# dordanino12/unet-convlstm

Hardware: AMD Instinct MI355X
Metric: training frames/sec, Moving-MNIST 64x64 seq-20 (higher is better)
Workload: dtype bf16; 1 GPU; TemporalUNetDualView(base_ch=64, use_skip_lstm=True) train step, 64x64 seq-20, per-GPU batch 32, AdamW+clip; global_batch=32, seq_len=20, parallelism=dp1

## Files before the change

### include/uclstm.h

```cpp
#ifndef UCLSTM_H
#define UCLSTM_H

#include <stdint.h>

#ifdef __cplusplus
extern "C" {
#endif

#define UCLSTM_ABI_VERSION 16

#define UCLSTM_OK            0
#define UCLSTM_E_BADARG     -1
#define UCLSTM_E_LAUNCH     -2
#define UCLSTM_E_NODEVICE   -3

#define UCLSTM_ACT_TYPE_BF16 0
#define UCLSTM_ACT_TYPE_F16  1


typedef struct {
    const void* ptr;
    int32_t C;
    int32_t Hs, Ws;
    int32_t offY, offX;
// ... 213 lines not shown
                             const int32_t* argmax, void* dx, float* dw, int32_t dw_accumulate, float* scratch, int32_t n_img,
                             int32_t H, int32_t W, int32_t Cp, int32_t C, int32_t k, void* stream);

int32_t uclstm_colsum(const void* a, float* out, int64_t pixels, int32_t Cp, void* stream);
int64_t uclstm_colsum_ordered_rows(int64_t pixels, int32_t Cp);
int32_t uclstm_colsum_ordered(const void* a, float* partials, float* out, int64_t pixels, int32_t Cp, int32_t accumulate,
                              int32_t act_type, void* stream);
int32_t uclstm_ordered_sum_f32(const float* partials, int32_t rows, int32_t cols, float* out, int32_t accumulate, void* stream);
int32_t uclstm_ordered_sum_f64(const double* partials, int32_t rows, int32_t cols, double* out, int32_t accumulate, void* stream);

int32_t uclstm_loss_fwd(const float* y_pred, const float* y, const float* mask, double* sums,
                        int64_t planes, int32_t H, int32_t W, void* stream);
int64_t uclstm_loss_fwd_ordered_rows(int64_t planes, int32_t H, int32_t W);
int32_t uclstm_loss_fwd_ordered(const float* y_pred, const float* y, const float* mask, double* partials, double* sums,
                                int32_t accumulate, int64_t planes, int32_t H, int32_t W, void* stream);
int32_t uclstm_loss_bwd(const float* y_pred, const float* y, const float* mask, const float* coefs,
                        float* grad, int64_t planes, int32_t H, int32_t W, void* stream);

int32_t uclstm_sumsq(const float* g, int64_t n, double* out , void* stream);
int64_t uclstm_sumsq_ordered_rows(int64_t n);
int32_t uclstm_sumsq_ordered(const float* g, int64_t n, double* partials, double* out, int32_t accumulate, void* stream);
int32_t uclstm_adamw_step(float* p, float* m, float* v, const float* g, int64_t n, const double* sumsq, float max_norm,
                          float lr, float beta1, float beta2, float eps, float weight_decay, int32_t step, void* stream);

int32_t uclstm_adamw_step_dev(float* p, float* m, float* v, const float* g, int64_t n, const double* sumsq, float* hyper, void* stream);

int32_t uclstm_adamw_step_groups(float* p, float* m, float* v, const float* g, int64_t n, const double* sumsq,
                                 const int64_t* runs, int32_t n_runs, float* hyper, int32_t n_groups,
                                 const float* scale_state, void* stream);

int32_t uclstm_adamw_step_scaled(float* p, float* m, float* v, const float* g, int64_t n, const double* sumsq, float max_norm,
                                 float lr, float beta1, float beta2, float eps, float weight_decay, const float* scale_state,
                                 void* stream);
int32_t uclstm_loss_scale_update(float* scale_state, const double* sumsq, float growth, float backoff, int32_t interval,
                                 void* stream);

int32_t uclstm_dataset_transform(const float* x_raw, const float* y_raw, float* x, float* y, float* mask, int64_t n_frames,
                                 int32_t C, int32_t HW, float norm_const, float min_vel, float max_vel, int32_t clip,
                                 float y_scale, float trans_min, float trans_max, void* stream);
int32_t uclstm_dataset_gather_transform(const float* x_all, const float* y_all, const int64_t* idx, int64_t n_seq, int64_t n_out,
                                        int32_t T, int32_t C, int32_t HW, float* x, float* y, float* mask, int32_t transform,
                                        float norm_const, float min_vel, float max_vel, int32_t clip, float y_scale,
                                        float trans_min, float trans_max, void* stream);
int32_t uclstm_dataset_gather_augment(const float* x_all, const float* y_all, const int64_t* idx, const int32_t* aug,
        int64_t n_seq, int64_t n_out, int32_t T_src, int32_t T_out, int32_t C, int32_t Hs, int32_t Ws, int32_t Ho, int32_t Wo,
        int32_t flags, float* x, float* y, float* mask, int32_t transform, float norm_const, float min_vel, float max_vel, int32_t clip,
// ... 81 lines not shown
```

### unet-convlstm_amd/_lib.py

```python
from __future__ import annotations

import ctypes as C
import os
import re

import torch

HERE = os.path.dirname(os.path.abspath(__file__))
LIB_PATH = os.environ.get("UCLSTM_LIB") or os.path.join(HERE, "libuclstm.so")
HEADER_PATH = os.path.join(HERE, "..", "include", "uclstm.h")

ABI_VERSION = 16
EPI_STORE, EPI_LSTM, EPI_ATOMIC = 0, 1, 2
NMODE_IDENTITY, NMODE_LSTM, NMODE_TAPMAJOR = 0, 1, 2
KMODE_IDENTITY, KMODE_GATES, KMODE_IM2COL = 0, 1, 2
ACT_TYPE_BF16, ACT_TYPE_F16 = 0, 1

_ERRORS = {-1: "bad argument (shape/alignment/null contract)", -2: "kernel launch failed", -3: "no gfx950 device"}


class UclstmError(RuntimeError):
    pass


# ... 120 lines not shown
    "uclstm_nchw_grad_to_nhwc": [_P, _P, _I, _I, _I, _I, _I, _P],
    "uclstm_im2col3x3_first": [_P, _P, _I, _I, _I, _I, _I, _I, _L, _L, _P],
    "uclstm_nchw_to_nhwc_f32": [_P, _P, _I, _I, _I, _I, _I, _P],
    "uclstm_nhwc_to_nchw_f32": [_P, _P, _I, _I, _I, _I, _I, _P],
    "uclstm_outconv_fwd": [_P, _P, _P, _P, _L, _I, _I, _I, _I, _P],
    "uclstm_outconv_bwd": [_P, _P, _P, _P, _P, _P, _L, _I, _I, _I, _I, _P],
    "uclstm_outconv_bwd_ordered_rows": [_L, _I],
    "uclstm_outconv_bwd_ordered": [_P, _P, _P, _P, _P, _P, _P, _I, _L, _I, _I, _I, _I, _I, _P],
    "uclstm_colsum": [_P, _P, _L, _I, _P],
    "uclstm_colsum_ordered_rows": [_L, _I],
    "uclstm_colsum_ordered": [_P, _P, _P, _L, _I, _I, _I, _P],
    "uclstm_ordered_sum_f32": [_P, _I, _I, _P, _I, _P],
    "uclstm_ordered_sum_f64": [_P, _I, _I, _P, _I, _P],
    "uclstm_attention_fwd": [_P, _P, _P, _P, _P, _P, _I, _I, _I, _I, _I, _I, _P],
    "uclstm_attention_bwd": [_P, _P, _P, _P, _P, _P, _P, _P, _I, _P, _I, _I, _I, _I, _I, _I, _P],
    "uclstm_loss_fwd": [_P, _P, _P, _P, _L, _I, _I, _P],
    "uclstm_loss_fwd_ordered_rows": [_L, _I, _I],
    "uclstm_loss_fwd_ordered": [_P, _P, _P, _P, _P, _I, _L, _I, _I, _P],
    "uclstm_loss_bwd": [_P, _P, _P, _P, _P, _L, _I, _I, _P],
    "uclstm_sumsq": [_P, _L, _P, _P],
    "uclstm_sumsq_ordered_rows": [_L],
    "uclstm_sumsq_ordered": [_P, _L, _P, _P, _I, _P],
    "uclstm_adamw_step": [_P, _P, _P, _P, _L, _P, _F, _F, _F, _F, _F, _F, _I, _P],
    "uclstm_adamw_step_dev": [_P, _P, _P, _P, _L, _P, _P, _P],
    "uclstm_adamw_step_groups": [_P, _P, _P, _P, _L, _P, _P, _I, _P, _I, _P, _P],
    "uclstm_adamw_step_scaled": [_P, _P, _P, _P, _L, _P, _F, _F, _F, _F, _F, _F, _P, _P],
    "uclstm_loss_scale_update": [_P, _P, _F, _F, _I, _P],
    "uclstm_dataset_transform": [_P, _P, _P, _P, _P, _L, _I, _I, _F, _F, _F, _I, _F, _F, _F, _P],
    "uclstm_dataset_gather_transform": [_P, _P, _P, _L, _L, _I, _I, _I, _P, _P, _P, _I, _F, _F, _F, _I, _F, _F, _F, _P],
    "uclstm_dataset_gather_augment": [_P, _P, _P, _P, _L, _L, _I, _I, _I, _I, _I, _I, _I, _I, _P, _P, _P, _I, _F, _F, _F, _I, _F, _F, _F, _P],
    "uclstm_plane_d4": [_P, _P, _L, _I, _I, _I, _I, _F, _P],
    "uclstm_sprites_render": [_P, _I, _I, _I, _P, _L, _I, _I, _I, _I, _I, _F, _P, _P, _P, _P, _P],
    "uclstm_metric_sums": [_P, _P, _P, _P, _L, _F, _F, _F, _P],
    "uclstm_metric_sums_ordered_rows": [_L],
    "uclstm_metric_sums_ordered": [_P, _P, _P, _P, _P, _I, _L, _F, _F, _F, _P],
    "uclstm_eval_stats": [C.POINTER(EvalDesc), _P],
    "uclstm_eval_stats_rows": [_L, _L],
    "uclstm_stream_spin": [_I, _P],
    "uclstm_abi_version": [],
    "uclstm_build_arch": [],
    "uclstm_source_hash": [],
    "uclstm_last_error_string": [],
}
_RESTYPES = {"uclstm_build_arch": C.c_char_p, "uclstm_source_hash": C.c_char_p, "uclstm_last_error_string": C.c_char_p, "uclstm_bn_bwd_reduce_rows": C.c_int64, "uclstm_bn_pool_bwd_rows": C.c_int64,
             "uclstm_eval_stats_rows": C.c_int64, "uclstm_colsum_ordered_rows": C.c_int64, "uclstm_outconv_bwd_ordered_rows": C.c_int64,
             "uclstm_loss_fwd_ordered_rows": C.c_int64, "uclstm_sumsq_ordered_rows": C.c_int64, "uclstm_metric_sums_ordered_rows": C.c_int64}
# ... 73 lines not shown
```

### unet-convlstm_amd/csrc/common.h

```cpp
#pragma once
#include <hip/hip_runtime.h>
#include <stdint.h>

#if defined(UCLSTM_ACT_F16)
#define uclstm_igemm_fwd uclstm_igemm_fwd_f16
#define uclstm_igemm_fwd_group uclstm_igemm_fwd_group_f16
#define uclstm_igemm_wgrad uclstm_igemm_wgrad_f16
#define uclstm_pack_weights uclstm_pack_weights_f16
#define uclstm_pack_weights_batched uclstm_pack_weights_batched_f16
#define uclstm_splitk_finish uclstm_splitk_finish_f16
#define uclstm_bn_apply_relu uclstm_bn_apply_relu_f16
#define uclstm_bn_bwd_reduce uclstm_bn_bwd_reduce_f16
#define uclstm_bn_bwd_apply uclstm_bn_bwd_apply_f16
#define uclstm_bn_head_fwd uclstm_bn_head_fwd_f16
#define uclstm_bn_apply_relu_pool uclstm_bn_apply_relu_pool_f16
#define uclstm_bn_pool_bwd_reduce uclstm_bn_pool_bwd_reduce_f16
#define uclstm_bn_pool_bwd_apply uclstm_bn_pool_bwd_apply_f16
#define uclstm_bn_head_bwd_reduce uclstm_bn_head_bwd_reduce_f16
#define uclstm_bn_head_bwd_apply uclstm_bn_head_bwd_apply_f16
#define uclstm_maxpool2_fwd uclstm_maxpool2_fwd_f16
#define uclstm_maxpool2_bwd uclstm_maxpool2_bwd_f16
#define uclstm_lstm_bwd_pointwise uclstm_lstm_bwd_pointwise_f16
#define uclstm_lstm_fwd_pointwise uclstm_lstm_fwd_pointwise_f16
#define uclstm_lstm_fwd_pointwise_group uclstm_lstm_fwd_pointwise_group_f16
#define uclstm_nchw_to_nhwc uclstm_nchw_to_nhwc_f16
#define uclstm_nhwc_to_nchw uclstm_nhwc_to_nchw_f16
#define uclstm_nchw_grad_to_nhwc uclstm_nchw_grad_to_nhwc_f16
#define uclstm_im2col3x3_first uclstm_im2col3x3_first_f16
#define uclstm_outconv_fwd uclstm_outconv_fwd_f16
#define uclstm_outconv_bwd uclstm_outconv_bwd_f16
#define uclstm_colsum uclstm_colsum_f16
#define uclstm_attention_fwd uclstm_attention_fwd_f16
// ... 101 lines not shown
```

### unet-convlstm_amd/csrc/loss_optim.hip

```cpp
#include "common.h"

namespace {

constexpr int NT = 256;

__device__ __forceinline__ double wave_sum(double v) {
#pragma unroll
    for (int o = 32; o > 0; o >>= 1) v += __shfl_xor(v, o, 64);
    return v;
}

template <int K>
__device__ __forceinline__ void block_sum(double (&v)[K], double* red ) {
#pragma unroll
    for (int k = 0; k < K; ++k) v[k] = wave_sum(v[k]);
    const int lane = threadIdx.x & 63, wave = threadIdx.x >> 6;
    if (lane == 0)
#pragma unroll
        for (int k = 0; k < K; ++k) red[wave * K + k] = v[k];
    __syncthreads();
    if (threadIdx.x == 0)
#pragma unroll
        for (int k = 0; k < K; ++k) v[k] = red[k] + red[K + k] + red[2 * K + k] + red[3 * K + k];
}
// ... 86 lines not shown
    const int64_t n4 = n >> 2;
    const float4* g4 = (const float4*)g;
    for (int64_t i = (int64_t)blockIdx.x * NT + threadIdx.x; i < n4; i += (int64_t)gridDim.x * NT) {
        const float4 v = g4[i];
        acc[0] += (double)(v.x * v.x + v.y * v.y) + (double)(v.z * v.z + v.w * v.w);
    }
    if (blockIdx.x == 0 && threadIdx.x < (n & 3)) {
        const float v = g[(n4 << 2) + threadIdx.x];
        acc[0] += (double)(v * v);
    }
    if constexpr (ORDERED) {
        block_sum_store<1>(acc, red, out + blockIdx.x);
    } else {
        block_sum<1>(acc, red);
        if (threadIdx.x == 0) atomicAdd(out, acc[0]);
    }
}

__device__ __forceinline__ bool step_overflowed(double ss) { return !(fabs(ss) <= 1.7976931348623157e308); }

__global__ void adamw_kernel(float* __restrict__ p, float* __restrict__ m, float* __restrict__ v, const float* __restrict__ g,
                             int64_t n, const double* __restrict__ sumsq, float max_norm, float lr, float b1, float b2, float eps,
                             float wd, float inv_bc1, float inv_sqrt_bc2) {
    float coef = 1.f;
    if (sumsq && max_norm > 0.f) {
        const float total = (float)sqrt(*sumsq);
        coef = fminf(max_norm / (total + 1e-6f), 1.f);
    }
    for (int64_t i = (int64_t)blockIdx.x * NT + threadIdx.x; i < n; i += (int64_t)gridDim.x * NT) {
        const float gi = g[i] * coef;
        float w = p[i] * (1.f - lr * wd);
        const float mi = b1 * m[i] + (1.f - b1) * gi;
        const float vi = b2 * v[i] + (1.f - b2) * gi * gi;
        const float denom = sqrtf(vi) * inv_sqrt_bc2 + eps;
        w -= lr * inv_bc1 * mi / denom;
        p[i] = w;
        m[i] = mi;
        v[i] = vi;
    }
}

__global__ void adamw_dev_kernel(float* __restrict__ p, float* __restrict__ m, float* __restrict__ v, const float* __restrict__ g,
                                 int64_t n, const double* __restrict__ sumsq, const float* __restrict__ hyper) {
    const float lr = hyper[0], b1 = hyper[1], b2 = hyper[2], eps = hyper[3], wd = hyper[4], max_norm = hyper[5];
    const double step = (double)hyper[6] + 1.0;
    const float inv_bc1 = (float)(1.0 / (1.0 - pow((double)b1, step)));
    const float inv_sqrt_bc2 = (float)(1.0 / sqrt(1.0 - pow((double)b2, step)));
    float coef = 1.f;
    if (sumsq && max_norm > 0.f) {
        const float total = (float)sqrt(*sumsq);
        coef = fminf(max_norm / (total + 1e-6f), 1.f);
    }
    for (int64_t i = (int64_t)blockIdx.x * NT + threadIdx.x; i < n; i += (int64_t)gridDim.x * NT) {
        const float gi = g[i] * coef;
        float w = p[i] * (1.f - lr * wd);
        const float mi = b1 * m[i] + (1.f - b1) * gi;
        const float vi = b2 * v[i] + (1.f - b2) * gi * gi;
        const float denom = sqrtf(vi) * inv_sqrt_bc2 + eps;
// ... 321 lines not shown
    const int64_t total = planes * H * W;
    if (total >= ((int64_t)1 << 31)) return UCLSTM_E_BADARG;
    UCLSTM_LAUNCH(loss_bwd_kernel, dim3(grid_for(total, 2048)), dim3(NT), 0, (hipStream_t)stream, y_pred, y, mask, coefs, grad,
                       total, make_fastdiv(H * W), make_fastdiv(W), H, W);
    return UCLSTM_OK;
}

extern "C" int32_t uclstm_sumsq(const float* g, int64_t n, double* out, void* stream) {
    if (!g || !out || n <= 0 || ((uintptr_t)g % 16)) return UCLSTM_E_BADARG;
    UCLSTM_LAUNCH(sumsq_kernel<false>, dim3(grid_for((n + 3) / 4, 1024)), dim3(NT), 0, (hipStream_t)stream, g, n, out);
    return UCLSTM_OK;
}

extern "C" int32_t uclstm_adamw_step(float* p, float* m, float* v, const float* g, int64_t n, const double* sumsq, float max_norm,
                                     float lr, float beta1, float beta2, float eps, float weight_decay, int32_t step, void* stream) {
    if (!p || !m || !v || !g || n <= 0 || step < 1) return UCLSTM_E_BADARG;
    const double bc1 = 1.0 - pow((double)beta1, (double)step);
    const double bc2 = 1.0 - pow((double)beta2, (double)step);
    UCLSTM_LAUNCH(adamw_kernel, dim3(grid_for(n, 2048)), dim3(NT), 0, (hipStream_t)stream, p, m, v, g, n, sumsq, max_norm, lr, beta1,
                       beta2, eps, weight_decay, (float)(1.0 / bc1), (float)(1.0 / sqrt(bc2)));
    return UCLSTM_OK;
}

extern "C" int32_t uclstm_adamw_step_dev(float* p, float* m, float* v, const float* g, int64_t n, const double* sumsq, float* hyper,
                                         void* stream) {
    if (!p || !m || !v || !g || n <= 0 || !hyper || ((uintptr_t)hyper % 16)) return UCLSTM_E_BADARG;
    UCLSTM_LAUNCH(adamw_dev_kernel, dim3(grid_for(n, 2048)), dim3(NT), 0, (hipStream_t)stream, p, m, v, g, n, sumsq, (const float*)hyper);
    UCLSTM_LAUNCH(adamw_advance_kernel, dim3(1), dim3(64), 0, (hipStream_t)stream, hyper);
    return UCLSTM_OK;
}

extern "C" int32_t uclstm_adamw_step_scaled(float* p, float* m, float* v, const float* g, int64_t n, const double* sumsq, float max_norm,
                                            float lr, float beta1, float beta2, float eps, float weight_decay, const float* scale_state,
                                            void* stream) {
    if (!p || !m || !v || !g || n <= 0 || !sumsq || !scale_state) return UCLSTM_E_BADARG;
    UCLSTM_LAUNCH(adamw_scaled_kernel, dim3(grid_for(n, 2048)), dim3(NT), 0, (hipStream_t)stream, p, m, v, g, n, sumsq, max_norm, lr, beta1,
                  beta2, eps, weight_decay, scale_state);
    return UCLSTM_OK;
}

extern "C" int32_t uclstm_adamw_step_groups(float* p, float* m, float* v, const float* g, int64_t n, const double* sumsq,
                                            const int64_t* runs, int32_t n_runs, float* hyper, int32_t n_groups,
                                            const float* scale_state, void* stream) {
    if (!p || !m || !v || !g || n <= 0 || !runs || n_runs <= 0 || !hyper || ((uintptr_t)hyper % 16) || n_groups <= 0 ||
        n_groups > 1024 || (scale_state && !sumsq))
        return UCLSTM_E_BADARG;
// ... 130 lines not shown
```

### unet-convlstm_amd/csrc/pack.hip

```cpp
#include "common.h"
#include <cstdlib>

namespace {

struct Decoded {
    bool valid;
    int64_t off;
};

struct PackDiv {
    FastDiv ktot, per_tap, n_cp, k_hdp, k_hd;
};
PackDiv make_pack_div(const uclstm_pack_desc& d) {
    PackDiv v;
    v.ktot = make_fastdiv((uint32_t)d.Ktot);
    v.per_tap = make_fastdiv((uint32_t)(d.kseg[0] + d.kseg[1]));
    v.n_cp = make_fastdiv((uint32_t)(d.n_cp > 0 ? d.n_cp : 1));
    v.k_hdp = make_fastdiv((uint32_t)(d.k_hdp > 0 ? d.k_hdp : 1));
    v.k_hd = make_fastdiv((uint32_t)(d.k_hd > 0 ? d.k_hd : 1));
    return v;
}

__device__ __forceinline__ bool decode_n(const uclstm_pack_desc& d, const PackDiv& dv, int n, int& n_ent, int& tapn) {
    tapn = 0;
// ... 281 lines not shown
    v.wp = (act16*)J.wp;
    v.lb = (int)blockIdx.x - J.block0;
    v.gx = J.gx;
    v.nblocks = J.nblocks;
    return v;
}
template <int TAPS>
__global__ __launch_bounds__(256) void pack_rows_batched_kernel(const uclstm_pack_job* __restrict__ jobs, int njobs) {
    const JobView v = find_job(jobs, njobs);
    const int by = v.lb / v.gx, bx = v.lb - by * v.gx;
    pack_rows_body<TAPS, false>(v.d, v.dv, v.w, v.wp, nullptr, 0, 0, nullptr, 0, (v.d.kseg[0] + 255) / 256, bx, by);
}
template <int TAPS>
__global__ __launch_bounds__(256) void pack_transposed_batched_kernel(const uclstm_pack_job* __restrict__ jobs, int njobs) {
    const JobView v = find_job(jobs, njobs);
    const int by = v.lb / v.gx, bx = v.lb - by * v.gx;
    pack_transposed_body<TAPS>(v.d, v.dv, v.w, v.wp, bx, by);
}
__global__ void pack_generic_batched_kernel(const uclstm_pack_job* __restrict__ jobs, int njobs) {
    const JobView v = find_job(jobs, njobs);
    pack_generic_body(v.d, v.dv, v.w, v.wp, (uint32_t)v.lb, (uint32_t)v.nblocks);
}

__global__ __launch_bounds__(256) void slab_fold_kernel(float* __restrict__ dwp, int nslab, int64_t slab, int64_t quads) {
    const int64_t q = (int64_t)blockIdx.x * 256 + threadIdx.x;
    if (q >= quads) return;
    float4* base = (float4*)dwp + q;
    const int64_t sq = slab / 4;
    float4 acc = base[0];
    int sl = 1;
    for (; sl + 8 <= nslab; sl += 8) {
        float4 t[8];
#pragma unroll
        for (int j = 0; j < 8; ++j) t[j] = base[(sl + j) * sq];
#pragma unroll
        for (int j = 0; j < 8; ++j) { acc.x += t[j].x; acc.y += t[j].y; acc.z += t[j].z; acc.w += t[j].w; }
    }
    for (; sl < nslab; ++sl) {
        const float4 t = base[sl * sq];
        acc.x += t.x; acc.y += t.y; acc.z += t.z; acc.w += t.w;
    }
    base[0] = acc;
}

__global__ void pack_bias_kernel(const uclstm_pack_desc d, const PackDiv dv, const float* __restrict__ b, float* __restrict__ bp) {
    const int n = blockIdx.x * blockDim.x + threadIdx.x;
// ... 89 lines not shown
    for (int i = 0; i < 5; ++i) {
        job->div[3 * i] = fs[i].magic;
        job->div[3 * i + 1] = fs[i].shift;
        job->div[3 * i + 2] = fs[i].d;
    }
    job->pad_ = 0;
    return job->family;
}
#endif

extern "C" int32_t uclstm_pack_weights_batched(const uclstm_pack_job* jobs_dev, int32_t njobs, int32_t family, int32_t total_blocks, void* stream) {
    if (!jobs_dev || njobs <= 0 || total_blocks <= 0 || family < 0 || family > 4) return UCLSTM_E_BADARG;
    hipStream_t st = (hipStream_t)stream;
    switch (family) {
        case 1: UCLSTM_LAUNCH(pack_rows_batched_kernel<9>, dim3(total_blocks), dim3(256), 0, st, jobs_dev, njobs); break;
        case 2: UCLSTM_LAUNCH(pack_rows_batched_kernel<4>, dim3(total_blocks), dim3(256), 0, st, jobs_dev, njobs); break;
        case 3: UCLSTM_LAUNCH(pack_transposed_batched_kernel<9>, dim3(total_blocks), dim3(256), 0, st, jobs_dev, njobs); break;
        case 4: UCLSTM_LAUNCH(pack_transposed_batched_kernel<4>, dim3(total_blocks), dim3(256), 0, st, jobs_dev, njobs); break;
        default: UCLSTM_LAUNCH(pack_generic_batched_kernel, dim3(total_blocks), dim3(256), 0, st, jobs_dev, njobs); break;
    }
    return UCLSTM_OK;
}

#ifndef UCLSTM_ACT_F16
static int generic_slab_groups(const uclstm_pack_desc& d, int nslab) {
    const int gx = grid_for((int64_t)d.N * d.Ktot);
    int gy = 1;
    if (nslab >= 16 && gx < 512) {
        gy = 1024 / gx;
        if (gy > nslab / 4) gy = nslab / 4;
        if (gy < 1) gy = 1;
    }
    return gy;
}
static int unpack_slab_groups(const uclstm_pack_desc& d, int nslab) {
    if (rows_family(d)) {
        if (nslab <= 64) return 1;
        if (((int64_t)d.N * d.Ktot % 4) == 0) return 1;
    }
    return generic_slab_groups(d, nslab);
}

static int32_t unpack_wgrad_impl(const uclstm_pack_desc* d, const float* dwp, int32_t nslab, int64_t slab, float* grad,
                                 int32_t accumulate, void* stream, bool split) {
    if (!desc_ok(d) || !dwp || !grad || nslab < 1 || (nslab > 1 && slab < (int64_t)d->N * d->Ktot)) return UCLSTM_E_BADARG;
    if (rows_family(*d) && nslab > 64 && (slab % 4) == 0 && ((int64_t)d->N * d->Ktot % 4) == 0 && ((uintptr_t)dwp % 16) == 0) {
// ... 57 lines not shown
```

### unet-convlstm_amd/ops.py

```python
from __future__ import annotations

import ctypes as C
import os
from typing import List, Optional, Sequence, Tuple

import torch

from . import _lib as L

BF16 = torch.bfloat16
F16 = torch.float16
F32 = torch.float32
ACT = (BF16, F16)

_COMPUTE_DTYPE = BF16


def set_compute_dtype(dtype) -> None:
    global _COMPUTE_DTYPE
    if dtype not in ACT:
        raise L.UclstmError(f"compute dtype must be torch.bfloat16 or torch.float16, got {dtype}")
    _COMPUTE_DTYPE = dtype


# ... 398 lines not shown
_ACTIVE_CACHE: Optional[PanelCache] = None


PREPACK = os.environ.get("UCLSTM_PREPACK", "1") != "0"
_PACK_PLAN: list = []
_PACK_READY: dict = {}
_PACK_RECORDING = False


PACK_BATCHED = os.environ.get("UCLSTM_PACK_BATCHED", "1") != "0"


PACK_SEGMENTS = tuple(float(x) for x in os.environ.get("UCLSTM_PACK_SEGMENTS", "0.02,0.08,0.2,0.35,0.5,0.65,0.8").split(",") if x)


def pack_segments(sizes: Sequence[int], fractions: Sequence[float]) -> List[int]:
    total, run, seg_of = float(sum(sizes)), 0, []
    for sz in sizes:
        seg_of.append(sum(1 for f in fractions if run >= f * total))
        run += sz
    return seg_of


class _PackBatch:

    def __init__(self, items):
        self.sig = tuple(key for key, _, _, _ in items)
        self.panels, self.keep, self.segments = {}, [], []
        dev = items[0][2].device
        seg_of = pack_segments([desc.N * desc.Ktot for _, desc, _, _ in items], PACK_SEGMENTS)
        jobs_all = []
        for n, seg in enumerate(sorted(set(seg_of))):
            groups: dict = {}
            for (key, desc, w, off), sg in zip(items, seg_of):
                if sg != seg:
                    continue
                wp = torch.empty((desc.N, desc.Ktot), dtype=key[3], device=dev)
                job = L.PackJob()
                fam = L.lib.uclstm_pack_job_init(C.byref(job), C.byref(desc), C.c_void_p(w.data_ptr() + 4 * off), _p(wp), 0)
                L.check(min(fam, 0), "pack_job_init")
                groups.setdefault((key[3], fam), []).append(job)
                self.panels[key] = (wp, n)
                self.keep.append(w)
            launches = []
            for (dtype, fam), jobs in groups.items():
                b0, first = 0, len(jobs_all)
                for j in jobs:
                    j.block0 = b0
                    b0 += j.nblocks
                    jobs_all.append(j)
                launches.append((dtype, fam, first * C.sizeof(L.PackJob), len(jobs), b0))
            self.segments.append(launches)
        arr = (L.PackJob * len(jobs_all))(*jobs_all)
        self.table = torch.frombuffer(bytearray(bytes(arr)), dtype=torch.uint8).to(dev)
        self.events: list = [None] * len(self.segments)

    def launch(self, side) -> None:
        base, st = self.table.data_ptr(), C.c_void_p(side.cuda_stream)
        for sg, launches in enumerate(self.segments):
            for dtype, fam, byte_off, n, blocks in launches:
                L.check(L.kernels(dtype).uclstm_pack_weights_batched(C.c_void_p(base + byte_off), n, fam, blocks, st), "pack_weights_batched")
            self.events[sg] = torch.cuda.Event()
            self.events[sg].record(side)

    def panel(self, key, main) -> torch.Tensor:
        wp, sg = self.panels[key]
        main.wait_event(self.events[sg])
        return wp


_PACK_BATCH: Optional[_PackBatch] = None


def prepack_begin() -> None:
    global _PACK_RECORDING, _PACK_PLAN, _PACK_BATCH
    _PACK_READY.clear()
    _PACK_RECORDING = False
    if not PREPACK:
        return
    plan, _PACK_PLAN = _PACK_PLAN, []
    _PACK_RECORDING = True
    if not plan:
        return
    dev = plan[0][2].device
    main, side = torch.cuda.current_stream(dev), side_stream(dev)
    if PACK_BATCHED:
        items, seen = [], set()
        for it in plan:
            if it[0] not in seen and it[2].data_ptr() == it[0][0]:
                seen.add(it[0])
                items.append(it)
        if not items:
            return
        if _PACK_BATCH is None or _PACK_BATCH.sig != tuple(it[0] for it in items):
            _PACK_BATCH = _PackBatch(items)
        side.wait_stream(main)
        _PACK_BATCH.launch(side)
        for key in _PACK_BATCH.panels:
            _PACK_READY[key] = _PACK_BATCH
        return
    side.wait_stream(main)
    with torch.cuda.stream(side):
        for key, desc, w, off in plan:
            if key in _PACK_READY or w.data_ptr() != key[0]:
                continue
            wp = torch.empty((desc.N, desc.Ktot), dtype=key[3], device=w.device)
            L.check(L.kernels(key[3]).uclstm_pack_weights(C.byref(desc), C.c_void_p(w.data_ptr() + 4 * off), _p(wp), _stream()), "pack_weights")
            wp.record_stream(main)
            ev = torch.cuda.Event()
            ev.record(side)
            _PACK_READY[key] = (wp, ev)


def prepack_end() -> None:
    global _PACK_RECORDING
    _PACK_READY.clear()
    _PACK_RECORDING = False


def pack_weights(desc: L.PackDesc, w: torch.Tensor, elem_offset: int = 0, dtype=BF16) -> torch.Tensor:
# ... 1419 lines not shown
```

### unet-convlstm_amd/optim.py

```python
from __future__ import annotations

import ctypes as C
from typing import Iterable, List, Optional, Sequence, Tuple

import torch


def build_run_table(sizes: Sequence[int], groups: Sequence[int]) -> List[Tuple[int, int, int]]:
    if len(sizes) != len(groups):
        raise ValueError("build_run_table: one group index per tensor")
    runs: List[Tuple[int, int, int]] = []
    off = 0
    for n, g in zip(sizes, groups):
        n, g = int(n), int(g)
        if n <= 0 or g < 0:
            raise ValueError("build_run_table: sizes must be positive and group indices non-negative")
        if runs and runs[-1][2] == g:
            runs[-1] = (runs[-1][0], off + n, g)
        else:
            runs.append((off, off + n, g))
        off += n
    return runs


# ... 176 lines not shown
            self.scale_state.copy_(fused["scale_state"])

    @torch.no_grad()
    def grad_norm(self) -> torch.Tensor:
        n = self.sumsq.sqrt()
        return n if self.scale_state is None else n / self._last_scale.double()

    def scale_loss(self, loss: torch.Tensor) -> torch.Tensor:
        return loss if self.scale_state is None else loss * self.scale_state[0]

    def _global_sumsq(self) -> None:
        from . import _lib as L
        from . import ops
        f = self.flat
        if ops.is_deterministic():
            partials = torch.empty(int(L.lib.uclstm_sumsq_ordered_rows(f.numel)), dtype=torch.float64, device=f.flat_g.device)
            ops._log_reduce("sumsq_ordered")
            L.check(L.lib.uclstm_sumsq_ordered(C.c_void_p(f.flat_g.data_ptr()), f.numel, C.c_void_p(partials.data_ptr()),
                                               C.c_void_p(self.sumsq.data_ptr()), 0, ops._stream()), "sumsq_ordered")
            return
        self.sumsq.zero_()
        ops._log_reduce("sumsq")
        L.check(L.lib.uclstm_sumsq(C.c_void_p(f.flat_g.data_ptr()), f.numel, C.c_void_p(self.sumsq.data_ptr()), ops._stream()), "sumsq")

    @torch.no_grad()
    def step(self, closure=None):
        from . import _lib as L
        from .ops import _stream
        assert closure is None
        g = self.param_groups[0]
        f = self.flat
        f.attach_grads()
        self.step_count += 1
        if self.uses_groups:
            if not torch.cuda.is_current_stream_capturing():
                self.sync_hyper()
            self._global_sumsq()
            state = None
            if self.scale_state is not None:
                self._last_scale.copy_(self.scale_state[0])
                state = C.c_void_p(self.scale_state.data_ptr())
            L.check(L.lib.uclstm_adamw_step_groups(C.c_void_p(f.flat_p.data_ptr()), C.c_void_p(self.m.data_ptr()), C.c_void_p(self.v.data_ptr()),
                                                   C.c_void_p(f.flat_g.data_ptr()), f.numel, C.c_void_p(self.sumsq.data_ptr()),
                                                   C.c_void_p(self.runs.data_ptr()), int(self.runs.shape[0]),
                                                   C.c_void_p(self.group_hyper.data_ptr()), len(self.param_groups), state, _stream()),
                    "adamw_step_groups")
# ... 11 lines not shown
                                                   float(self.max_grad_norm or 0.0), float(g["lr"]), float(g["betas"][0]), float(g["betas"][1]),
                                                   float(g["eps"]), float(g["weight_decay"]), C.c_void_p(self.scale_state.data_ptr()), _stream()),
                    "adamw_step_scaled")
            gr, bo, it = self._scale_cfg
            L.check(L.lib.uclstm_loss_scale_update(C.c_void_p(self.scale_state.data_ptr()), C.c_void_p(self.sumsq.data_ptr()), gr, bo, it,
                                                   _stream()), "loss_scale_update")
            from . import ops
            ops.weights_changed()
            return None
        if self.capturable:
            if not torch.cuda.is_current_stream_capturing():
                self.sync_hyper()
            self._global_sumsq()
            L.check(L.lib.uclstm_adamw_step_dev(C.c_void_p(f.flat_p.data_ptr()), C.c_void_p(self.m.data_ptr()), C.c_void_p(self.v.data_ptr()),
                                                C.c_void_p(f.flat_g.data_ptr()), f.numel, C.c_void_p(self.sumsq.data_ptr()),
                                                C.c_void_p(self.hyper.data_ptr()), _stream()), "adamw_step_dev")
            from . import ops
            ops.weights_changed()
            return None
        sq = None
        if self.max_grad_norm is not None:
            self._global_sumsq()
            sq = C.c_void_p(self.sumsq.data_ptr())
        L.check(L.lib.uclstm_adamw_step(C.c_void_p(f.flat_p.data_ptr()), C.c_void_p(self.m.data_ptr()), C.c_void_p(self.v.data_ptr()),
                                        C.c_void_p(f.flat_g.data_ptr()), f.numel, sq,
                                        float(self.max_grad_norm or 0.0), float(g["lr"]), float(g["betas"][0]), float(g["betas"][1]),
                                        float(g["eps"]), float(g["weight_decay"]), self.step_count, _stream()), "adamw_step")
        from . import ops
        ops.weights_changed()
        return None
```

Measured before the change: 20640 frames/s.

## Fuse AdamW update with bf16 weight panel packing for 3x3 conv weights

Adds a kernel that applies the AdamW update to 9-tap conv weights and writes the packed low-precision GEMM panel in the same pass. A ranges kernel updates the remaining parameters. On the next forward, the pack launch skips the fused panels when a version token shows the weights are unchanged. This removes a separate re-read of the fp32 weights for packing and the side-stream event waits on those panels. The cost is extra bookkeeping (run tables, a binary search per element, reuse tokens) and a risk of stale panels if the token check misses a weight change.

```diff
diff --git a/include/uclstm.h b/include/uclstm.h
--- a/include/uclstm.h
+++ b/include/uclstm.h
@@ -259,6 +259,16 @@
 int32_t uclstm_sumsq_ordered(const float* g, int64_t n, double* partials, double* out, int32_t accumulate, void* stream);
 int32_t uclstm_adamw_step(float* p, float* m, float* v, const float* g, int64_t n, const double* sumsq, float max_norm,
                           float lr, float beta1, float beta2, float eps, float weight_decay, int32_t step, void* stream);
+
+int32_t uclstm_adamw_pack_step(const uclstm_pack_job* jobs_dev, int32_t njobs, int32_t total_blocks, float* p, float* m, float* v,
+                               const float* g, int64_t n, const double* sumsq, float max_norm, float lr, float beta1, float beta2,
+                               float eps, float weight_decay, int32_t step, void* stream);
+int32_t uclstm_adamw_pack_step_f16(const uclstm_pack_job* jobs_dev, int32_t njobs, int32_t total_blocks, float* p, float* m, float* v,
+                                   const float* g, int64_t n, const double* sumsq, float max_norm, float lr, float beta1, float beta2,
+                                   float eps, float weight_decay, int32_t step, void* stream);
+int32_t uclstm_adamw_step_ranges(float* p, float* m, float* v, const float* g, int64_t n, const int64_t* ranges_dev, int32_t n_ranges,
+                                 int64_t total, const double* sumsq, float max_norm, float lr, float beta1, float beta2, float eps,
+                                 float weight_decay, int32_t step, void* stream);
 
 int32_t uclstm_adamw_step_dev(float* p, float* m, float* v, const float* g, int64_t n, const double* sumsq, float* hyper, void* stream);
 
diff --git a/unet-convlstm_amd/_lib.py b/unet-convlstm_amd/_lib.py
--- a/unet-convlstm_amd/_lib.py
+++ b/unet-convlstm_amd/_lib.py
@@ -166,6 +166,9 @@
     "uclstm_sumsq_ordered_rows": [_L],
     "uclstm_sumsq_ordered": [_P, _L, _P, _P, _I, _P],
     "uclstm_adamw_step": [_P, _P, _P, _P, _L, _P, _F, _F, _F, _F, _F, _F, _I, _P],
+    "uclstm_adamw_pack_step": [_P, _I, _I, _P, _P, _P, _P, _L, _P, _F, _F, _F, _F, _F, _F, _I, _P],
+    "uclstm_adamw_pack_step_f16": [_P, _I, _I, _P, _P, _P, _P, _L, _P, _F, _F, _F, _F, _F, _F, _I, _P],
+    "uclstm_adamw_step_ranges": [_P, _P, _P, _P, _L, _P, _I, _L, _P, _F, _F, _F, _F, _F, _F, _I, _P],
     "uclstm_adamw_step_dev": [_P, _P, _P, _P, _L, _P, _P, _P],
     "uclstm_adamw_step_groups": [_P, _P, _P, _P, _L, _P, _P, _I, _P, _I, _P, _P],
     "uclstm_adamw_step_scaled": [_P, _P, _P, _P, _L, _P, _F, _F, _F, _F, _F, _F, _P, _P],
diff --git a/unet-convlstm_amd/csrc/adamw_update.h b/unet-convlstm_amd/csrc/adamw_update.h
--- /dev/null
+++ b/unet-convlstm_amd/csrc/adamw_update.h
@@ -0,0 +1,43 @@
+#pragma once
+#include "common.h"
+
+struct AdamwCoef {
+    float coef;
+    float b1, omb1;
+    float b2, omb2;
+    float eps;
+    float decay;
+    float lr_bc1;
+    float inv_sqrt_bc2;
+};
+
+__device__ __forceinline__ AdamwCoef adamw_coef(const double* __restrict__ sumsq, float max_norm, float lr, float b1, float b2, float eps,
+                                                float wd, float inv_bc1, float inv_sqrt_bc2) {
+#pragma clang fp contract(off)
+    AdamwCoef c;
+    c.coef = 1.f;
+    if (sumsq && max_norm > 0.f) {
+        const float total = (float)sqrt(*sumsq);
+        c.coef = fminf(max_norm / (total + 1e-6f), 1.f);
+    }
+    c.b1 = b1;
+    c.omb1 = 1.f - b1;
+    c.b2 = b2;
+    c.omb2 = 1.f - b2;
+    c.eps = eps;
+    c.decay = __builtin_fmaf(-lr, wd, 1.f);
+    c.lr_bc1 = lr * inv_bc1;
+    c.inv_sqrt_bc2 = inv_sqrt_bc2;
+    return c;
+}
+
+__device__ __forceinline__ void adamw_update(const AdamwCoef& c, float g, float& p, float& m, float& v) {
+#pragma clang fp contract(off)
+    const float gi = g * c.coef;
+    const float mi = __builtin_fmaf(c.omb1, gi, c.b1 * m);
+    const float vi = c.b2 * v + (c.omb2 * gi) * gi;
+    const float denom = __builtin_fmaf(sqrtf(vi), c.inv_sqrt_bc2, c.eps);
+    p = c.decay * p - (c.lr_bc1 * mi) / denom;
+    m = mi;
+    v = vi;
+}
diff --git a/unet-convlstm_amd/csrc/common.h b/unet-convlstm_amd/csrc/common.h
--- a/unet-convlstm_amd/csrc/common.h
+++ b/unet-convlstm_amd/csrc/common.h
@@ -8,6 +8,7 @@
 #define uclstm_igemm_wgrad uclstm_igemm_wgrad_f16
 #define uclstm_pack_weights uclstm_pack_weights_f16
 #define uclstm_pack_weights_batched uclstm_pack_weights_batched_f16
+#define uclstm_adamw_pack_step uclstm_adamw_pack_step_f16
 #define uclstm_splitk_finish uclstm_splitk_finish_f16
 #define uclstm_bn_apply_relu uclstm_bn_apply_relu_f16
 #define uclstm_bn_bwd_reduce uclstm_bn_bwd_reduce_f16
diff --git a/unet-convlstm_amd/csrc/loss_optim.hip b/unet-convlstm_amd/csrc/loss_optim.hip
--- a/unet-convlstm_amd/csrc/loss_optim.hip
+++ b/unet-convlstm_amd/csrc/loss_optim.hip
@@ -1,4 +1,5 @@
 #include "common.h"
+#include "adamw_update.h"
 
 namespace {
 
@@ -132,18 +133,31 @@
 __global__ void adamw_kernel(float* __restrict__ p, float* __restrict__ m, float* __restrict__ v, const float* __restrict__ g,
                              int64_t n, const double* __restrict__ sumsq, float max_norm, float lr, float b1, float b2, float eps,
                              float wd, float inv_bc1, float inv_sqrt_bc2) {
-    float coef = 1.f;
-    if (sumsq && max_norm > 0.f) {
-        const float total = (float)sqrt(*sumsq);
-        coef = fminf(max_norm / (total + 1e-6f), 1.f);
-    }
+    const AdamwCoef c = adamw_coef(sumsq, max_norm, lr, b1, b2, eps, wd, inv_bc1, inv_sqrt_bc2);
     for (int64_t i = (int64_t)blockIdx.x * NT + threadIdx.x; i < n; i += (int64_t)gridDim.x * NT) {
-        const float gi = g[i] * coef;
-        float w = p[i] * (1.f - lr * wd);
-        const float mi = b1 * m[i] + (1.f - b1) * gi;
-        const float vi = b2 * v[i] + (1.f - b2) * gi * gi;
-        const float denom = sqrtf(vi) * inv_sqrt_bc2 + eps;
-        w -= lr * inv_bc1 * mi / denom;
+        float w = p[i], mi = m[i], vi = v[i];
+        adamw_update(c, g[i], w, mi, vi);
+        p[i] = w;
+        m[i] = mi;
+        v[i] = vi;
+    }
+}
+
+__global__ void adamw_ranges_kernel(float* __restrict__ p, float* __restrict__ m, float* __restrict__ v, const float* __restrict__ g,
+                                    int64_t n, const int64_t* __restrict__ ranges, int n_ranges, int64_t total,
+                                    const double* __restrict__ sumsq, float max_norm, float lr, float b1, float b2, float eps, float wd,
+                                    float inv_bc1, float inv_sqrt_bc2) {
+    const AdamwCoef c = adamw_coef(sumsq, max_norm, lr, b1, b2, eps, wd, inv_bc1, inv_sqrt_bc2);
+    for (int64_t j = (int64_t)blockIdx.x * NT + threadIdx.x; j < total; j += (int64_t)gridDim.x * NT) {
+        int r = 0;
+        for (int hi = n_ranges - 1; r < hi;) {
+            const int mid = (r + hi + 1) >> 1;
+            if (ranges[3 * mid + 2] <= j) r = mid; else hi = mid - 1;
+        }
+        const int64_t i = ranges[3 * r] + (j - ranges[3 * r + 2]);
+        if (i < 0 || i >= ranges[3 * r + 1] || i >= n) continue;
+        float w = p[i], mi = m[i], vi = v[i];
+        adamw_update(c, g[i], w, mi, vi);
         p[i] = w;
         m[i] = mi;
         v[i] = vi;
@@ -511,6 +525,19 @@
     return UCLSTM_OK;
 }
 
+extern "C" int32_t uclstm_adamw_step_ranges(float* p, float* m, float* v, const float* g, int64_t n, const int64_t* ranges_dev,
+                                            int32_t n_ranges, int64_t total, const double* sumsq, float max_norm, float lr, float beta1,
+                                            float beta2, float eps, float weight_decay, int32_t step, void* stream) {
+    if (!p || !m || !v || !g || n <= 0 || step < 1 || n_ranges < 0 || total < 0 || total > n || (total > 0 && (!ranges_dev || n_ranges < 1)))
+        return UCLSTM_E_BADARG;
+    if (total == 0) return UCLSTM_OK;
+    const double bc1 = 1.0 - pow((double)beta1, (double)step);
+    const double bc2 = 1.0 - pow((double)beta2, (double)step);
+    UCLSTM_LAUNCH(adamw_ranges_kernel, dim3(grid_for(total, 2048)), dim3(NT), 0, (hipStream_t)stream, p, m, v, g, n, ranges_dev, n_ranges, total,
+                  sumsq, max_norm, lr, beta1, beta2, eps, weight_decay, (float)(1.0 / bc1), (float)(1.0 / sqrt(bc2)));
+    return UCLSTM_OK;
+}
+
 extern "C" int32_t uclstm_adamw_step_dev(float* p, float* m, float* v, const float* g, int64_t n, const double* sumsq, float* hyper,
                                          void* stream) {
     if (!p || !m || !v || !g || n <= 0 || !hyper || ((uintptr_t)hyper % 16)) return UCLSTM_E_BADARG;
diff --git a/unet-convlstm_amd/csrc/pack.hip b/unet-convlstm_amd/csrc/pack.hip
--- a/unet-convlstm_amd/csrc/pack.hip
+++ b/unet-convlstm_amd/csrc/pack.hip
@@ -1,4 +1,5 @@
 #include "common.h"
+#include "adamw_update.h"
 #include <cstdlib>
 
 namespace {
@@ -327,6 +328,80 @@
     pack_generic_body(v.d, v.dv, v.w, v.wp, (uint32_t)v.lb, (uint32_t)v.nblocks);
 }
 
+template <int TAPS>
+__global__ __launch_bounds__(256) void adamw_pack_rows_kernel(const uclstm_pack_job* __restrict__ jobs, int njobs, float* __restrict__ p,
+                                                              float* __restrict__ m, float* __restrict__ v, const float* __restrict__ g,
+                                                              int64_t n_elems, const double* __restrict__ sumsq, float max_norm, float lr,
+                                                              float b1, float b2, float eps, float wd, float inv_bc1, float inv_sqrt_bc2) {
+    __shared__ float buf[256 * TAPS + 32];
+    const JobView J = find_job(jobs, njobs);
+    const uclstm_pack_desc& d = J.d;
+    const int n = J.lb / J.gx, bx = J.lb - n * J.gx;
+    const int chunks0 = (d.kseg[0] + 255) / 256;
+    const int s = bx >= chunks0 ? 1 : 0;
+    const int c0 = (bx - (s ? chunks0 : 0)) * 256;
+    const int seg = s ? d.kseg[1] : d.kseg[0];
+    const int per_tap = d.kseg[0] + d.kseg[1];
+    int n_ent, tapn;
+    const bool ok_n = decode_n(d, J.dv, n, n_ent, tapn);
+    int nval = (s ? d.cvalid[1] : d.cvalid[0]) - c0;
+    nval = nval < 0 ? 0 : (nval > 256 ? 256 : nval);
+    int count = ok_n ? nval * TAPS : 0;
+    const int64_t off = (int64_t)(J.w - p) + (int64_t)n_ent * d.stride_n + (int64_t)tapn * d.stride_ntap +
+                        (int64_t)((s ? d.choff[1] : d.choff[0]) + c0) * TAPS;
+    if (off < 0 || off + count > n_elems) count = 0;
+    const AdamwCoef c = adamw_coef(sumsq, max_norm, lr, b1, b2, eps, wd, inv_bc1, inv_sqrt_bc2);
+    {
+        float gv[TAPS], pv[TAPS], mv[TAPS], vv[TAPS];
+#pragma unroll
+        for (int i = 0; i < TAPS; ++i) {
+            const int e = i * 256 + threadIdx.x;
+            const int64_t a = e < count ? off + e : 0;
+            gv[i] = g[a];
+            pv[i] = p[a];
+            mv[i] = m[a];
+            vv[i] = v[a];
+        }
+#pragma unroll
+        for (int i = 0; i < TAPS; ++i) {
+            const int e = i * 256 + threadIdx.x;
+            adamw_update(c, gv[i], pv[i], mv[i], vv[i]);
+            if (e < count) {
+                const int64_t a = off + e;
+                p[a] = pv[i];
+                m[a] = mv[i];
+                v[a] = vv[i];
+                buf[e + (e / TAPS >> 3)] = pv[i];
+            }
+        }
+    }
+    __syncthreads();
+    act16* wp = J.wp;
+    const int64_t pbase = (int64_t)n * d.Ktot + (s ? d.kseg[0] : 0) + c0;
+    const bool vec = ((d.kseg[0] | d.kseg[1]) & 7) == 0 && ((uintptr_t)wp & 15) == 0;
+    const int nv = count ? nval : 0;
+    for (int item = threadIdx.x; item < TAPS * 32; item += 256) {
+        const int t = item >> 5, g8 = item & 31;
+        const int cl = g8 * 8;
+        if (c0 + cl >= seg) continue;
+        const int ts = d.tap_flip ? TAPS - 1 - t : t;
+        float x[8];
+#pragma unroll
+        for (int j = 0; j < 8; ++j) x[j] = buf[(cl + j) * TAPS + ts + g8];
+        act16x8 o;
+#pragma unroll
+        for (int j = 0; j < 8; ++j) o[j] = f32_to_act(cl + j < nv ? x[j] : 0.f);
+        act16* dst = wp + pbase + (int64_t)t * per_tap + cl;
+        if (vec) {
+            *(act16x8*)dst = o;
+        } else {
+#pragma unroll
+            for (int j = 0; j < 8; ++j)
+                if (c0 + cl + j < seg) dst[j] = o[j];
+        }
+    }
+}
+
 __global__ __launch_bounds__(256) void slab_fold_kernel(float* __restrict__ dwp, int nslab, int64_t slab, int64_t quads) {
     const int64_t q = (int64_t)blockIdx.x * 256 + threadIdx.x;
     if (q >= quads) return;
@@ -462,6 +537,17 @@
     return UCLSTM_OK;
 }
 
+extern "C" int32_t uclstm_adamw_pack_step(const uclstm_pack_job* jobs_dev, int32_t njobs, int32_t total_blocks, float* p, float* m, float* v,
+                                          const float* g, int64_t n, const double* sumsq, float max_norm, float lr, float beta1, float beta2,
+                                          float eps, float weight_decay, int32_t step, void* stream) {
+    if (!jobs_dev || njobs <= 0 || total_blocks <= 0 || !p || !m || !v || !g || n <= 0 || step < 1) return UCLSTM_E_BADARG;
+    const double bc1 = 1.0 - pow((double)beta1, (double)step);
+    const double bc2 = 1.0 - pow((double)beta2, (double)step);
+    UCLSTM_LAUNCH(adamw_pack_rows_kernel<9>, dim3(total_blocks), dim3(256), 0, (hipStream_t)stream, jobs_dev, njobs, p, m, v, g, n, sumsq,
+                  max_norm, lr, beta1, beta2, eps, weight_decay, (float)(1.0 / bc1), (float)(1.0 / sqrt(bc2)));
+    return UCLSTM_OK;
+}
+
 #ifndef UCLSTM_ACT_F16
 static int generic_slab_groups(const uclstm_pack_desc& d, int nslab) {
     const int gx = grid_for((int64_t)d.N * d.Ktot);
diff --git a/unet-convlstm_amd/ops.py b/unet-convlstm_amd/ops.py
--- a/unet-convlstm_amd/ops.py
+++ b/unet-convlstm_amd/ops.py
@@ -444,11 +444,65 @@
     return seg_of
 
 
+FUSE_OPT_PACK = os.environ.get("UCLSTM_FUSE_OPT_PACK", "1") != "0"
+FAM_ROWS9 = 1
+
+
+def rows_job_runs(desc) -> Optional[List[Tuple[int, int]]]:
+    taps = int(desc.taps)
+    if desc.k_mode != L.KMODE_IDENTITY or desc.stride_tap != 1 or desc.stride_k != taps:
+        return None
+    if desc.n_mode == L.NMODE_IDENTITY:
+        rows, fits = int(desc.n_valid), desc.N >= desc.n_valid
+    elif desc.n_mode == L.NMODE_LSTM:
+        rows, fits = 4 * int(desc.n_valid), desc.N >= 64 * ((desc.n_valid + 15) // 16)
+    else:
+        return None
+    srcs = [s for s in range(int(desc.nsrc)) if desc.cvalid[s] > 0]
+    if not fits or rows <= 0 or not srcs or any(desc.cvalid[s] > desc.kseg[s] for s in srcs):
+        return None
+    return [(r * int(desc.stride_n) + int(desc.choff[s]) * taps, r * int(desc.stride_n) + int(desc.choff[s] + desc.cvalid[s]) * taps)
+            for r in range(rows) for s in srcs]
+
+
+def merge_runs(runs: Sequence[Tuple[int, int]]) -> Optional[List[Tuple[int, int]]]:
+    out: List[Tuple[int, int]] = []
+    for b, e in sorted(runs):
+        if e <= b:
+            continue
+        if out and b < out[-1][1]:
+            return None
+        if out and b == out[-1][1]:
+            out[-1] = (out[-1][0], e)
+        else:
+            out.append((b, e))
+    return out
+
+
+def complement_ranges(covered: Sequence[Tuple[int, int]], n: int) -> List[Tuple[int, int, int]]:
+    out, at, before = [], 0, 0
+    for b, e in covered:
+        if b < at or e > n:
+            raise ValueError(f"complement_ranges: [{b}, {e}) is not sorted, disjoint and inside [0, {n})")
+        if b > at:
+            out.append((at, b, before))
+            before += b - at
+        at = e
+    if at < n:
+        out.append((at, n, before))
+    return out
+
+
+def fused_reuse_ok(token, epoch: int, version: int, sig, stream: int) -> bool:
+    return token is not None and token == (epoch, version, sig, stream)
+
+
 class _PackBatch:
 
     def __init__(self, items):
         self.sig = tuple(key for key, _, _, _ in items)
         self.panels, self.keep, self.segments = {}, [], []
+        self._jobs: list = []
         dev = items[0][2].device
         seg_of = pack_segments([desc.N * desc.Ktot for _, desc, _, _ in items], PACK_SEGMENTS)
         jobs_all = []
@@ -464,6 +518,7 @@
                 groups.setdefault((key[3], fam), []).append(job)
                 self.panels[key] = (wp, n)
                 self.keep.append(w)
+                self._jobs.append((key, job, w))
             launches = []
             for (dtype, fam), jobs in groups.items():
                 b0, first = 0, len(jobs_all)
@@ -473,13 +528,89 @@
                     jobs_all.append(j)
                 launches.append((dtype, fam, first * C.sizeof(L.PackJob), len(jobs), b0))
             self.segments.append(launches)
+        self._plan_fusion(jobs_all)
         arr = (L.PackJob * len(jobs_all))(*jobs_all)
         self.table = torch.frombuffer(bytearray(bytes(arr)), dtype=torch.uint8).to(dev)
         self.events: list = [None] * len(self.segments)
 
-    def launch(self, side) -> None:
+    def _plan_fusion(self, jobs_all) -> None:
+        self.fuse_keys: set = set()
+        self.fuse_tables: dict = {}
+        self.fuse_runs: List[Tuple[int, int]] = []
+        self.fuse_weights: list = []
+        self.segments_rest = self.segments
+        self.fused_token, self.fused_live, self._fuse_plan = None, False, None
+        claimed: dict = {}
+        per_dtype: dict = {}
+        sz = C.sizeof(L.PackJob)
+        for key, job, w in self._jobs:
+            if job.family != FAM_ROWS9:
+                continue
+            runs = rows_job_runs(job.d)
+            chans = [(job.d.choff[s], job.d.choff[s] + job.d.cvalid[s]) for s in range(job.d.nsrc) if job.d.cvalid[s] > 0]
+            mine = claimed.setdefault((key[0], key[1]), [])
+            if runs is None or any(a < d and c < b for a, b in chans for c, d in mine):
+                continue
+            mine.extend(chans)
+            self.fuse_keys.add(key)
+            self.fuse_weights.append(w)
+            self.fuse_runs.extend((job.w + 4 * b, job.w + 4 * e) for b, e in runs)
+            per_dtype.setdefault(key[3], []).append(job)
+        if not self.fuse_keys:
+            return
+        by_id = {id(job): key for key, job, _ in self._jobs}
+        rest = []
+        for launches in self.segments:
+            out = []
+            for dtype, fam, byte_off, n, blocks in launches:
+                first = byte_off // sz
+                jobs = jobs_all[first:first + n]
+                keep = [j for j in jobs if by_id[id(j)] not in self.fuse_keys]
+                if len(keep) == len(jobs):
+                    out.append((dtype, fam, byte_off, n, blocks))
+                elif keep:
+                    out.append((dtype, fam, len(jobs_all) * sz, len(keep), self._append_rebased(jobs_all, keep)))
+            rest.append(out)
+        self.segments_rest = rest
+        for dtype, jobs in per_dtype.items():
+            first = len(jobs_all)
+            self.fuse_tables[dtype] = (first * sz, len(jobs), self._append_rebased(jobs_all, jobs))
+
+    @staticmethod
+    def _append_rebased(jobs_all, jobs) -> int:
+        b0 = 0
+        for j in jobs:
+            c = L.PackJob()
+            C.memmove(C.byref(c), C.byref(j), C.sizeof(L.PackJob))
+            c.block0 = b0
+            b0 += c.nblocks
+            jobs_all.append(c)
+        return b0
+
+    def fuse_plan(self, flat_p: torch.Tensor):
+        if not self.fuse_keys:
+            return None
+        ident = (flat_p.data_ptr(), flat_p.numel())
+        if self._fuse_plan is None or self._fuse_plan[0] != ident:
+            base, n, plan = ident[0], ident[1], None
+            rel = [((b - base) // 4, (e - base) // 4) for b, e in self.fuse_runs]
+            if all(0 <= b and e <= n for b, e in rel):
+                covered = merge_runs(rel)
+                if covered is not None:
+                    table = complement_ranges(covered, n)
+                    dev_t = torch.tensor(table or [(0, 0, 0)], dtype=torch.int64).to(flat_p.device)
+                    plan = (dev_t, len(table), sum(e - b for b, e, _ in table))
+            self._fuse_plan = (ident, plan, flat_p)
+        return self._fuse_plan[1]
+
+    def fuse_version(self) -> int:
+        flat_p = self._fuse_plan[2]
+        return int(flat_p._version) + sum(int(w._version) for w in self.fuse_weights)
+
+    def launch(self, side, skip_fused: bool = False) -> None:
         base, st = self.table.data_ptr(), C.c_void_p(side.cuda_stream)
-        for sg, launches in enumerate(self.segments):
+        self.fused_live = bool(skip_fused)
+        for sg, launches in enumerate(self.segments_rest if skip_fused else self.segments):
             for dtype, fam, byte_off, n, blocks in launches:
                 L.check(L.kernels(dtype).uclstm_pack_weights_batched(C.c_void_p(base + byte_off), n, fam, blocks, st), "pack_weights_batched")
             self.events[sg] = torch.cuda.Event()
@@ -487,7 +618,8 @@
 
     def panel(self, key, main) -> torch.Tensor:
         wp, sg = self.panels[key]
-        main.wait_event(self.events[sg])
+        if not (self.fused_live and key in self.fuse_keys):
+            main.wait_event(self.events[sg])
         return wp
 
 
@@ -517,7 +649,10 @@
         if _PACK_BATCH is None or _PACK_BATCH.sig != tuple(it[0] for it in items):
             _PACK_BATCH = _PackBatch(items)
         side.wait_stream(main)
-        _PACK_BATCH.launch(side)
+        b = _PACK_BATCH
+        reuse = (FUSE_OPT_PACK and b.fused_token is not None
+                 and fused_reuse_ok(b.fused_token, WEIGHTS_EPOCH, b.fuse_version(), b.sig, main.cuda_stream))
+        _PACK_BATCH.launch(side, skip_fused=reuse)
         for key in _PACK_BATCH.panels:
             _PACK_READY[key] = _PACK_BATCH
         return
diff --git a/unet-convlstm_amd/optim.py b/unet-convlstm_amd/optim.py
--- a/unet-convlstm_amd/optim.py
+++ b/unet-convlstm_amd/optim.py
@@ -222,6 +222,31 @@
         self.sumsq.zero_()
         ops._log_reduce("sumsq")
         L.check(L.lib.uclstm_sumsq(C.c_void_p(f.flat_g.data_ptr()), f.numel, C.c_void_p(self.sumsq.data_ptr()), ops._stream()), "sumsq")
+
+    def _step_with_panels(self, sq, g) -> bool:
+        from . import _lib as L
+        from . import ops
+        batch = ops._PACK_BATCH
+        if not ops.FUSE_OPT_PACK or batch is None:
+            return False
+        f = self.flat
+        plan = batch.fuse_plan(f.flat_p)
+        if plan is None:
+            return False
+        ranges, n_ranges, total = plan
+        st = ops._stream()
+        hyper = (float(self.max_grad_norm or 0.0), float(g["lr"]), float(g["betas"][0]), float(g["betas"][1]), float(g["eps"]),
+                 float(g["weight_decay"]), self.step_count, st)
+        bufs = (C.c_void_p(f.flat_p.data_ptr()), C.c_void_p(self.m.data_ptr()), C.c_void_p(self.v.data_ptr()), C.c_void_p(f.flat_g.data_ptr()),
+                f.numel)
+        base = batch.table.data_ptr()
+        for dtype, (byte_off, njobs, blocks) in batch.fuse_tables.items():
+            fn = L.lib.uclstm_adamw_pack_step if dtype == torch.bfloat16 else L.lib.uclstm_adamw_pack_step_f16
+            L.check(fn(C.c_void_p(base + byte_off), njobs, blocks, *bufs, sq, *hyper), "adamw_pack_step")
+        L.check(L.lib.uclstm_adamw_step_ranges(*bufs, C.c_void_p(ranges.data_ptr()), n_ranges, total, sq, *hyper), "adamw_step_ranges")
+        ops.weights_changed()
+        batch.fused_token = (ops.WEIGHTS_EPOCH, batch.fuse_version(), batch.sig, torch.cuda.current_stream(f.flat_p.device).cuda_stream)
+        return True
 
     @torch.no_grad()
     def step(self, closure=None):
@@ -279,6 +304,8 @@
         if self.max_grad_norm is not None:
             self._global_sumsq()
             sq = C.c_void_p(self.sumsq.data_ptr())
+        if self._step_with_panels(sq, g):
+            return None
         L.check(L.lib.uclstm_adamw_step(C.c_void_p(f.flat_p.data_ptr()), C.c_void_p(self.m.data_ptr()), C.c_void_p(self.v.data_ptr()),
                                         C.c_void_p(f.flat_g.data_ptr()), f.numel, sq,
                                         float(self.max_grad_norm or 0.0), float(g["lr"]), float(g["betas"][0]), float(g["betas"][1]),
```

New measurement: 20750 frames/s (median of 6 runs). Within noise of the previous version (+0.5%).
